# lbcb-sci/raven

Hardware: AMD Instinct MI355X
Metric: read Gbase/s through overlap+polish (higher is better)
Workload: dtype u32

## Files before the change

raven_amd/csrc/poa4.hip:

```cpp
#include <algorithm>
#include <cstddef>
#include <cstdio>
#include <cstdlib>
#include <cstring>
#include <vector>

#include "poa.h"
#include "poa2_window.h"

namespace rvn {

namespace {

struct P4 {
  static constexpr int G = 4, GS = 16, kBand = 32;
  static constexpr int kRing = 22;
  static constexpr int kRowB = 64;
  static constexpr int kMaxD = 8;
  static constexpr int kEdges = 8;
  static constexpr int kEdgesMax = 15;
  static constexpr int kU = 8;
};
constexpr u32 kNone4 = 0xFFFFu;
constexpr i32 kNegU = -0x30000000;
// ... 93 lines not shown
__host__ __device__ __forceinline__ i32 sext16(u32 x) { return static_cast<i32>(static_cast<i16>(x & 0xFFFFu)); }
__host__ __device__ __forceinline__ i32 imax(i32 a, i32 b) { return a > b ? a : b; }
__host__ __device__ __forceinline__ i32 imin(i32 a, i32 b) { return a < b ? a : b; }
template <bool HI>
__host__ __device__ __forceinline__ u32 add_half(u32 a, u32 p) {
#if defined(__HIP_DEVICE_COMPILE__)
  u32 d;
  if constexpr (HI)
    asm("v_add_u32_sdwa %0, %1, %2 dst_sel:DWORD dst_unused:UNUSED_PAD src0_sel:DWORD src1_sel:WORD_1" : "=v"(d) : "v"(a), "v"(p));
  else
    asm("v_add_u32_sdwa %0, %1, %2 dst_sel:DWORD dst_unused:UNUSED_PAD src0_sel:DWORD src1_sel:WORD_0" : "=v"(d) : "v"(a), "v"(p));
  return d;
#else
  return a + (HI ? p >> 16 : p & 0xFFFFu);
#endif
}
template <bool HI, int TAG>
__host__ __device__ __forceinline__ i32 cell_key(u32 w) {
#if defined(__HIP_DEVICE_COMPILE__)
  i32 d;
  if constexpr (HI) asm("v_mad_i32_i16 %0, %1, %2, %3 op_sel:[1,0,0,0]" : "=v"(d) : "v"(w), "s"(256), "n"(TAG));
  else asm("v_mad_i32_i16 %0, %1, %2, %3" : "=v"(d) : "v"(w), "s"(256), "n"(TAG));
  return d;
#else
  return static_cast<i32>(static_cast<i16>((HI ? w >> 16 : w) & 0xFFFFu)) * 256 + TAG;
#endif
}
__host__ __device__ __forceinline__ u32 keys_to_pair(i32 k0, i32 k1) {
#if defined(__HIP_DEVICE_COMPILE__)
  return __builtin_amdgcn_perm(static_cast<u32>(k1), static_cast<u32>(k0), 0x06050201u);
#else
  return ((static_cast<u32>(k0) >> 8) & 0xFFFFu) | ((static_cast<u32>(k1) >> 8) << 16);
#endif
}
__host__ __device__ __forceinline__ i32 imax3(i32 a, i32 b, i32 c) {
  const i32 m = a > b ? a : b;
  return m > c ? m : c;
}
template <int B>
__host__ __device__ __forceinline__ u32 put_byte(u32 acc, u32 v) {
#if defined(__HIP_DEVICE_COMPILE__)
  constexpr u32 sel = B == 0 ? 0x0C0C0C04u : (B == 1 ? 0x0C0C0400u : (B == 2 ? 0x0C040100u : 0x04020100u));
  return __builtin_amdgcn_perm(v, acc, sel);
#else
  const u32 keep = B == 0 ? 0u : (B == 1 ? 0xFFu : (B == 2 ? 0xFFFFu : 0xFFFFFFu));
  return (acc & keep) | ((v & 0xFFu) << (8 * B));
#endif
}
__host__ __device__ __forceinline__ u32 pack16(i32 lo, i32 hi) {
#if defined(__HIP_DEVICE_COMPILE__)
  return __builtin_amdgcn_perm(static_cast<u32>(hi), static_cast<u32>(lo), 0x05040100u);
#else
  return (static_cast<u32>(lo) & 0xFFFFu) | (static_cast<u32>(hi) << 16);
#endif
}
__host__ __device__ __forceinline__ u32 clamp_pair(u32 w) {
#if defined(__HIP_DEVICE_COMPILE__)
  typedef short pk16 __attribute__((ext_vector_type(2)));
  const pk16 lim = {static_cast<short>(kNegInf16), static_cast<short>(kNegInf16)};
  return __builtin_bit_cast(u32, __builtin_elementwise_max(__builtin_bit_cast(pk16, w), lim));
#else
  const i32 a = sext16(w), b = sext16(w >> 16);
  return pack16(a < kNegInf16 ? kNegInf16 : a, b < kNegInf16 ? kNegInf16 : b);
#endif
}
__host__ __device__ __forceinline__ u32 lds_ld32(const Poa4Lds& S, u32 off) {
  return *reinterpret_cast<const u32*>(reinterpret_cast<const unsigned char*>(&S) + off);
}
__host__ __device__ __forceinline__ void lds_st32(Poa4Lds& S, u32 off, u32 v) {
  *reinterpret_cast<u32*>(reinterpret_cast<unsigned char*>(&S) + off) = v;
}
__host__ __device__ __forceinline__ i32 lds_ld16(const Poa4Lds& S, u32 off) {
  return *reinterpret_cast<const i16*>(reinterpret_cast<const unsigned char*>(&S) + off);
}
__host__ __device__ __forceinline__ void lds_order() {
#if defined(__HIP_DEVICE_COMPILE__)
  __builtin_amdgcn_wave_barrier();
#else
  sv::sync();
#endif
}
#if defined(__HIP_DEVICE_COMPILE__)
#define P4_MARK(x) asm volatile("; P4MARK " x)
#define P4_ASSUME_GLOBAL(p) \
  __builtin_assume(!__builtin_amdgcn_is_shared((const void*)(p))); \
  __builtin_assume(!__builtin_amdgcn_is_private((const void*)(p)))
#define P4_ASSUME_LDS(p) __builtin_assume(__builtin_amdgcn_is_shared((const void*)(p)))
#else
#define P4_MARK(x)
#define P4_ASSUME_GLOBAL(p)
#define P4_ASSUME_LDS(p)
#endif

__host__ __device__ __forceinline__ unsigned char* opaque(unsigned char* p) {
#if defined(__HIP_DEVICE_COMPILE__)
  asm volatile("" : "+v"(p));
#endif
  return p;
}

__host__ __device__ inline u32 group_min_u(u32 v) {
#pragma unroll
  for (int off = 8; off > 0; off >>= 1) {
    const u32 o = static_cast<u32>(sv::bperm(static_cast<int>(v), sv::lane() ^ off));
    v = o < v ? o : v;
  }
  return v;
}
__host__ __device__ inline i32 group_max_i(i32 v) {
#pragma unroll
  for (int off = 8; off > 0; off >>= 1) {
    const i32 o = sv::bperm(v, sv::lane() ^ off);
    v = o > v ? o : v;
  }
  return v;
}

__host__ __device__ inline u32 poa4_nth_pred_rank(const Poa4Slot& sl, u32 v, u32 k, bool full) {
  const Poa2Slot& g = sl.g;
  const u32 c = g.in_cnt[v];
  u32 seen = 0;
  for (u32 i = 0; i < c; ++i) {
    const u32 t = g.in_tail[v * kPoaMaxIn + i];
    if (full || g.mark[t]) {
      if (seen == k) return sl.rb[t] & 0xFFFFu;
      ++seen;
    }
  }
  return 0;
}

__host__ __device__ __forceinline__ u32 mulhi_u32(u32 a, u32 b) {
#if defined(__HIP_DEVICE_COMPILE__)
  return __umulhi(a, b);
#else
  return static_cast<u32>((static_cast<unsigned long long>(a) * b) >> 32);
#endif
}
__host__ __device__ __forceinline__ u32 magic_of(u32 d) { return d <= 1 ? 0u : static_cast<u32>(0x100000000ULL / d) + 1u; }
__host__ __device__ __forceinline__ u32 div_magic(u32 n, u32 m) { return m ? mulhi_u32(n, m) : n; }

struct alignas(16) Poa4LdsDesc {
  u32 segtab[32];
  u32 seq2[60];
  u8 bytes[1024];
};

__host__ __device__ inline void poa4_guide_to_lds(Poa4LdsDesc& S, const PoaLayer* Lp, u32 len, i32 span) {
  const int lane = sv::lane();
  if (lane < 8) {
    const i32 sg = lane;
    const i32 x0 = (sg * span) / 8, x1 = ((sg + 1) * span) / 8;
    const i32 wa = sg == 0 ? 0 : static_cast<i32>(Lp->way[sg - 1]);
    const i32 wb = sg == 7 ? static_cast<i32>(len) : static_cast<i32>(Lp->way[sg]);
    S.segtab[4 * sg] = static_cast<u32>(x0);
    S.segtab[4 * sg + 1] = static_cast<u32>(wa);
    S.segtab[4 * sg + 2] = static_cast<u32>(wb - wa);
    S.segtab[4 * sg + 3] = magic_of(static_cast<u32>(x1 > x0 ? x1 - x0 : 1));
  }
}
template <class K>
__host__ __device__ __forceinline__ i32 poa4_band_start(const Poa4LdsDesc& S, i32 bpos, i32 lb, i32 span, u32 span_magic, u32 len) {
  i32 x = bpos - lb;
  x = x < 0 ? 0 : (x > span ? span : x);
  const u32 seg = div_magic(static_cast<u32>(x) * 8u, span_magic);
  const u32 sg = seg > 7u ? 7u : seg;
  const uint4 st = *reinterpret_cast<const uint4*>(&S.segtab[4 * sg]);
  const i32 dw = static_cast<i32>(st.z);
  const u32 num = static_cast<u32>(x - static_cast<i32>(st.x)) * static_cast<u32>(dw < 0 ? -dw : dw);
  const i32 qn = static_cast<i32>(div_magic(num, st.w));
  i32 b = static_cast<i32>(st.y) + (dw < 0 ? -qn : qn) - K::kBand / 2;
  const i32 bmax = static_cast<i32>(len) + 1 - K::kBand;
// ... 749 lines not shown
              g.al[static_cast<size_t>(kt[u][k]) * 4 + ac[u]] = static_cast<u16>(id);
              g.al_cnt[kt[u][k]] = static_cast<u8>(ac[u] + 1);
              if (c2 == 0) mine.x = kt[u][k];
              else if (c2 == 1) mine.x |= kt[u][k] << 16;
              else mine.y = kt[u][k];
              ++c2;
            }
          }
          if (ac[u] < 4) {
            g.al[static_cast<size_t>(an[u]) * 4 + ac[u]] = static_cast<u16>(id);
            g.al_cnt[an[u]] = static_cast<u8>(ac[u] + 1);
          }
          if (c2 == 0) mine.x = an[u];
          else if (c2 == 1) mine.x |= an[u] << 16;
          else if (c2 == 2) mine.y = an[u];
          else mine.y |= an[u] << 16;
          ++c2;
        }
        *reinterpret_cast<uint2*>(g.al + static_cast<size_t>(id) * 4) = mine;
        g.al_cnt[id] = static_cast<u8>(c2);
      }
      if (why == 0) total_new += cnt;
      tgt[u] = t;
    }
    u32 icnt[UP];
    uint4 ta[UP], tb[UP];
#pragma unroll
    for (int u = 0; u < UP; ++u) {
      const bool old = valid[u] && why == 0 && !is_new[u];
      const u32 t = old ? tgt[u] : 0u;
      icnt[u] = old ? g.in_cnt[t] : 0u;
      ta[u] = old ? *reinterpret_cast<const uint4*>(g.in_tail + static_cast<size_t>(t) * kPoaMaxIn) : uint4{0, 0, 0, 0};
      tb[u] = old ? *reinterpret_cast<const uint4*>(g.in_tail + static_cast<size_t>(t) * kPoaMaxIn + 8) : uint4{0, 0, 0, 0};
    }
#pragma unroll
    for (int u = 0; u < UP; ++u) {
      const u32 last_t = static_cast<u32>(sv::bperm(static_cast<int>(u == 0 ? prev_tgt : tgt[u > 0 ? u - 1 : 0]), gbase | (GW - 1)));
      const i32 last_w = sv::bperm(u == 0 ? prev_w : wgt[u > 0 ? u - 1 : 0], gbase | (GW - 1));
      const u32 tail = static_cast<u32>(shift1(static_cast<int>(tgt[u]), static_cast<int>(last_t)));
      const i32 tw = shift1(wgt[u], last_w);
      if (valid[u] && why == 0) {
        const u32 head = tgt[u];
        if (len >= 2) {
          if (is_new[u]) g.visits[head] = 1;
          else atomic_inc_u16(g.visits, head);
        }
        if (p[u] >= 1) {
          const i32 weight = tw + wgt[u];
          const u32 c = icnt[u];
          u32 found = 0xFFu;
#pragma unroll
          for (int i2 = 0; i2 < 16; ++i2) {
            const uint4& src4 = i2 < 8 ? ta[u] : tb[u];
            const u32 wd = (i2 & 7) < 2 ? src4.x : ((i2 & 7) < 4 ? src4.y : ((i2 & 7) < 6 ? src4.z : src4.w));
            const u32 tt = (wd >> (16 * (i2 & 1))) & 0xFFFFu;
            if (static_cast<u32>(i2) < c && tt == tail && found == 0xFFu) found = static_cast<u32>(i2);
          }
          if (found != 0xFFu) {
            atomic_add_i32(g.in_w + static_cast<size_t>(head) * kPoaMaxIn + found, weight);
          } else if (c >= static_cast<u32>(kPoaMaxIn)) {
            why = 3;
          } else {
            g.in_tail[static_cast<size_t>(head) * kPoaMaxIn + c] = static_cast<u16>(tail);
            g.in_w[static_cast<size_t>(head) * kPoaMaxIn + c] = weight;
            g.in_cnt[head] = static_cast<u8>(c + 1);
            atomic_inc_u16(g.out_cnt, tail);
          }
        }
      }
    }
    {
      const u32 wmax = static_cast<u32>(gmax(static_cast<i32>(why)));
      why = wmax;
    }
    prev_tgt = static_cast<u32>(sv::bperm(static_cast<int>(tgt[UP - 1]), gbase | (GW - 1)));
    prev_w = sv::bperm(wgt[UP - 1], gbase | (GW - 1));
  }
  t_add += sv::clock() - t0;
  t0 = sv::clock();
  const u32 n_new = total_new;
  lds_order();
  const bool doit = act && why == 0 && n_new != 0;
  if (sv::any(doit)) {
    const u32 max_old = static_cast<u32>(sv::wave_max(doit ? static_cast<int>(n_old) : 0));
    for (u32 r0 = 0; r0 < max_old; r0 += UP * GW) {
      u32 rr[UP], vv[UP];
#pragma unroll
      for (int u = 0; u < UP; ++u) {
        rr[u] = r0 + static_cast<u32>(GW) * static_cast<u32>(u) + static_cast<u32>(gl);
        vv[u] = (doit && rr[u] < n_old) ? g.order[rr[u]] : 0u;
      }
#pragma unroll
      for (int u = 0; u < UP; ++u) {
        if (doit && rr[u] < n_old) {
          u32 lo = 0, hi = n_new;
          while (lo < hi) {
            const u32 mid = (lo + hi) >> 1;
            if (nslot[mid] <= rr[u]) lo = mid + 1;
            else hi = mid;
          }
          g.order2[rr[u] + lo] = static_cast<u16>(vv[u]);
          rb16[2 * static_cast<size_t>(vv[u])] = static_cast<u16>(rr[u] + lo);
        }
      }
    }
    const u32 max_new = static_cast<u32>(sv::wave_max(doit ? static_cast<int>(n_new) : 0));
    for (u32 t = static_cast<u32>(gl); t < max_new; t += GW) {
      if (doit && t < n_new) {
        const u32 r = static_cast<u32>(nslot[t]) + t;
        g.order2[r] = static_cast<u16>(n_old + t);
        rb16[2 * static_cast<size_t>(n_old + t)] = static_cast<u16>(r);
      }
    }
    if (doit) flip = !flip;
  }
  if (act && why == 0) nn = n_old + n_new;
  sv::sync();
  t_ord += sv::clock() - t0;
  return why;
}

__host__ __device__ inline void poa4_consensus_general(Poa2Slot& g, u32 n_nodes, u32 nmax, const PoaWindow& win, int trim, Poa4Lds& S,
                                               u8* out, u32* out_len) {
  const int lane = sv::lane();
  for (u32 r = lane; r < n_nodes; r += 64) g.rank_of[g.order[r]] = static_cast<u16>(r);
  constexpr u32 kCap = sizeof(Poa4Lds) / 4;
  i32* lsc = reinterpret_cast<i32*>(&S);
  i32 maxn = -1;
  if (n_nodes > kCap) {
    if (lane == 0) maxn = poa_consensus_scores_lane0(g, n_nodes);
    maxn = sv::rfl(maxn);
  } else {
    i32 max_sc = 0;
    const u32 nn = n_nodes;
    for (u32 r0 = 0; r0 < nn; r0 += 64) {
      const u32 rows = nn - r0 < 64 ? nn - r0 : 64;
      int m_it = 0, m_c = 0, m_t01 = 0, m_t23 = 0, m_w0 = 0, m_w1 = 0, m_w2 = 0, m_w3 = 0;
      if (static_cast<u32>(lane) < rows) {
        m_it = g.order[r0 + lane];
        m_c = g.in_cnt[m_it];
        const u16* tp = g.in_tail + static_cast<size_t>(m_it) * kPoaMaxIn;
        const i32* wp = g.in_w + static_cast<size_t>(m_it) * kPoaMaxIn;
        m_t01 = static_cast<int>(static_cast<u32>(tp[0]) | (static_cast<u32>(tp[1]) << 16));
        m_t23 = static_cast<int>(static_cast<u32>(tp[2]) | (static_cast<u32>(tp[3]) << 16));
        m_w0 = wp[0];
        m_w1 = wp[1];
        m_w2 = wp[2];
        m_w3 = wp[3];
      }
      for (u32 l = 0; l < rows; ++l) {
        const int li = static_cast<int>(l);
        const u32 it = static_cast<u32>(sv::rl(m_it, li));
        const u32 c = static_cast<u32>(sv::rl(m_c, li));
        const u32 t01 = static_cast<u32>(sv::rl(m_t01, li)), t23 = static_cast<u32>(sv::rl(m_t23, li));
        const i32 w0 = sv::rl(m_w0, li), w1 = sv::rl(m_w1, li), w2 = sv::rl(m_w2, li), w3 = sv::rl(m_w3, li);
        i32 sc = -1, pd = -1, pd_sc = 0;
        for (u32 k = 0; k < c; ++k) {
          i32 wgt, t;
          if (k < 4) {
            t = static_cast<i32>(((k < 2 ? t01 : t23) >> (16 * (k & 1))) & 0xFFFFu);
            wgt = k == 0 ? w0 : (k == 1 ? w1 : (k == 2 ? w2 : w3));
          } else {
            wgt = g.in_w[static_cast<size_t>(it) * kPoaMaxIn + k];
            t = static_cast<i32>(g.in_tail[static_cast<size_t>(it) * kPoaMaxIn + k]);
          }
          const i32 st = lsc[t];
          if (sc < wgt || (sc == wgt && pd_sc <= st)) {
            sc = wgt;
            pd = t;
            pd_sc = st;
          }
        }
        if (pd != -1) sc += pd_sc;
        lds_order();
        if (lane == 0) {
          lsc[it] = sc;
          g.scores[it] = sc;
          g.preds[it] = pd;
        }
        lds_order();
        if (maxn == -1 || max_sc < sc) {
          maxn = static_cast<i32>(it);
          max_sc = sc;
        }
      }
    }
  }
  sv::sync();
  u32 cl = 0;
  i32 begin = 0, end = -1;
  if (lane == 0) poa_consensus_trace_lane0(g, n_nodes, nmax, win, trim, maxn, &cl, &begin, &end);
  cl = static_cast<u32>(sv::rfl(static_cast<int>(cl)));
  begin = sv::rfl(begin);
  end = sv::rfl(end);
  sv::sync();
  i32 n_out = end - begin + 1;
  if (n_out < 0) n_out = 0;
  if (static_cast<u32>(n_out) > win.out_cap) n_out = static_cast<i32>(win.out_cap);
  for (i32 p = lane; p < n_out; p += 64) out[p] = g.code[g.stack[cl - 1 - static_cast<u32>(begin + p)]];
// ... 358 lines not shown
    me.phase = kFailed;
    me.status = 4;
    if (lane == 0) C.st[rec] = me;
    return;
  }
  const Poa4Slot sl = poa4_carve(poa4_slot_of(A, C, wave_dp, q), A.nmax, A.lmax);
  Poa2Slot g = sl.g;
  for (u32 i = lane; i < L.len; i += 64) {
    S.bytes[i] = static_cast<u8>(poa_layer_code(A.src, L, i));
    g.pos_node[i] = static_cast<u16>(kNone4);
  }
  lds_order();
  if (lane < 60) {
    u32 x = 0;
    for (u32 c = 0; c < 16; ++c) {
      const i32 p = static_cast<i32>(static_cast<u32>(lane) * 16 + c) - 1;
      if (p >= 0 && p < static_cast<i32>(L.len)) x |= static_cast<u32>(S.bytes[p] & 3u) << (2 * c);
    }
    sl.seq2g[lane] = x;
  }
  const u32 blen = A.layers[wq.layer_first].len;
  const u32 offset = static_cast<u32>(0.01 * blen);
  const bool full = L.begin < offset && L.end > blen - offset;
  u32 r_lo = 0, r_hi = me.nn;
  if (!full) {
    lds_order();
    poa4_subgraph_marks(g, sl.rb, me.flip ? g.order2 : g.order, reinterpret_cast<u32*>(S.bytes), me.nn, L.begin, L.end, r_lo, r_hi);
  }
  const i32 lb = static_cast<i32>(L.begin), span = static_cast<i32>(L.end) - static_cast<i32>(L.begin) + 1;
  poa4_guide_to_lds(S, A.layers + wq.layer_first + liq, L.len, span);
  lds_order();
  if (lane < 32) sl.seq2g[64 + lane] = S.segtab[lane];
  u32 b_first = 0;
  if (r_hi > r_lo) {
    const u32 v0 = (me.flip ? g.order2 : g.order)[r_lo];
    b_first = static_cast<u32>(poa4_band_start<K>(S, static_cast<i32>(sl.rb[v0] >> 16), lb, span,
                                                   magic_of(static_cast<u32>(span > 0 ? span : 1)), L.len));
  }
  me.act = 1;
  me.full = full ? 1u : 0u;
  me.len = L.len;
  me.lb = L.begin;
  me.span = static_cast<u32>(span);
  me.r_lo = r_lo;
  me.n_rows = r_hi - r_lo;
  me.t_end = 0;
  me.best_rho1 = 0;
  me.b_first = b_first;
  me.dflag = 0;
  if (lane == 0) C.st[rec] = me;
  if (A.phase_cycles && lane == 0) sv::atomic_add(&A.phase_cycles[0], sv::clock() - t0);
}

constexpr int kDescPer = 4;
template <class K>
__host__ __device__ inline void poa4_phase_desc_onewave(const Poa4Args& A, const Poa4Ctx& C, Poa4LdsDesc& S, u32 rec) {
  const int lane = sv::lane();
  const u32 wave_dp = rec / P4::G;
  const int q = static_cast<int>(rec % P4::G);
  if (poa4_my_record(C, wave_dp, q) == 0xFFFFFFFFu) return;
  const Poa4Slot sl = poa4_carve(poa4_slot_of(A, C, wave_dp, q), A.nmax, A.lmax);
  const Poa2Slot& g = sl.g;
  const Poa4Win me = C.st[rec];
  if (me.phase != kRunning || !me.act) return;
  const unsigned long long t_desc0 = sv::clock();
  const u32 nn = me.nn;
  const bool full = me.full != 0;
  const u32 len = me.len, r_lo = me.r_lo, n_rows = me.n_rows, r_hi = r_lo + n_rows;
  const i32 lb = static_cast<i32>(me.lb), span = static_cast<i32>(me.span), b_first = static_cast<i32>(me.b_first);
  const u32 span_magic = magic_of(static_cast<u32>(span > 0 ? span : 1));
  const u32 dump_off = poa4_dump_byte(q);
  const u32 neg_off = poa4_neg_byte(q);
  const u32 neg2 = neg_off | (neg_off << 16);
  u32 flag = 0, marked_rows = 0;
  i32 t_end = 0;
  {
    const u32 gw = sl.seq2g[lane < 60 ? lane : 64 + (lane - 60)];
    const u32 gw2 = lane < 28 ? sl.seq2g[68 + lane] : 0u;
    if (lane < 60) S.seq2[lane] = gw;
    else S.segtab[lane - 60] = gw;
    if (lane < 28) S.segtab[4 + lane] = gw2;
  }
  lds_order();
  for (u32 v0 = 0; v0 < nn; v0 += 64 * kDescPer) {
    u32 rbv[kDescPer];
#pragma unroll
    for (int u = 0; u < kDescPer; ++u) {
      const u32 v = v0 + static_cast<u32>(u) * 64 + static_cast<u32>(lane);
      rbv[u] = v < nn ? sl.rb[v] : 0u;
    }
#pragma unroll
    for (int u = 0; u < kDescPer; ++u) {
      const u32 v = v0 + static_cast<u32>(u) * 64 + static_cast<u32>(lane);
      if (v < nn) {
        const i32 b = poa4_band_start<K>(S, static_cast<i32>(rbv[u] >> 16), lb, span, span_magic, len);
        sl.rbl[v] = (rbv[u] & 0xFFFFu) | (static_cast<u32>(b) << 16);
      }
    }
  }
  sv::sync();
  for (u32 v0 = 0; v0 < nn; v0 += 64 * kDescPer) {
    u32 vv[kDescPer], rbv[kDescPer], cc[kDescPer], code[kDescPer], outc_f[kDescPer], outc_s[kDescPer], mk[kDescPer];
    uint4 tl[kDescPer];
#pragma unroll
    for (int u = 0; u < kDescPer; ++u) {
      vv[u] = v0 + static_cast<u32>(u) * 64 + static_cast<u32>(lane);
      const u32 vq = vv[u] < nn ? vv[u] : 0u;
      rbv[u] = sl.rbl[vq];
      cc[u] = g.in_cnt[vq];
      code[u] = g.code[vq];
      outc_f[u] = g.out_cnt[vq];
      outc_s[u] = full ? 0u : g.sub_out[vq];
      mk[u] = full ? 1u : g.mark[vq];
      tl[u] = *reinterpret_cast<const uint4*>(g.in_tail + static_cast<size_t>(vq) * kPoaMaxIn);
    }
    bool ok[kDescPer], marked[kDescPer];
    u32 cmax = 0;
#pragma unroll
    for (int u = 0; u < kDescPer; ++u) {
      const u32 r = rbv[u] & 0xFFFFu;
      ok[u] = vv[u] < nn && r >= r_lo && r < r_hi;
      marked[u] = ok[u] && mk[u] != 0;
      if (!marked[u]) cc[u] = 0;
      cmax = cc[u] > cmax ? cc[u] : cmax;
    }
    cmax = static_cast<u32>(sv::wave_max(static_cast<i32>(cmax)));
    u32 trb[kDescPer][8], tmk[kDescPer][8];
#pragma unroll
    for (int k = 0; k < 8; ++k) {
      if (static_cast<u32>(k) < cmax) {
#pragma unroll
        for (int u = 0; u < kDescPer; ++u) {
          const u32 wd = k < 2 ? tl[u].x : (k < 4 ? tl[u].y : (k < 6 ? tl[u].z : tl[u].w));
          const u32 t = static_cast<u32>(k) < cc[u] ? (wd >> (16 * (k & 1))) & 0xFFFFu : 0u;
          trb[u][k] = sl.rbl[t];
          tmk[u][k] = full ? 1u : g.mark[t];
        }
      } else {
#pragma unroll
        for (int u = 0; u < kDescPer; ++u) {
          trb[u][k] = 0;
          tmk[u][k] = 0;
        }
      }
    }
#pragma unroll
    for (int u = 0; u < kDescPer; ++u) {
      const u32 v = vv[u];
      const u32 r = rbv[u] & 0xFFFFu;
      const i32 b = static_cast<i32>(rbv[u] >> 16);
      const u32 rho = r - r_lo;
      u32 ep[4] = {neg2, neg2, neg2, neg2};
      u32 np = 0, lbw = 0, lbk7 = 0;
      auto edge = [&](u32 rbt, bool inside) {
        if (!inside) return;
        const u32 lbk = r - (rbt & 0xFFFFu);
        const i32 d = b - static_cast<i32>(rbt >> 16);
        if (lbk < 1 || lbk > static_cast<u32>(K::kRing - 1) || lbk > rho || d < 0 || d > K::kMaxD) {
          flag = 7;
        } else if (np < static_cast<u32>(K::kEdges)) {
          const u32 e = poa4_ring_byte(q, ((rho - lbk) % static_cast<u32>(K::kRing)) * static_cast<u32>(kRowW4));
          const u32 idx = np >> 1;
          const u32 keep = (np & 1) ? 0x0000FFFFu : 0xFFFF0000u;
          const u32 put = (np & 1) ? e << 16 : e;
#pragma unroll
          for (u32 i = 0; i < 4; ++i) ep[i] = i == idx ? ((ep[i] & keep) | put) : ep[i];
          if (np < 6) lbw |= lbk << (5 * np);
          if (np == 7) lbk7 = lbk;
        } else if (np < static_cast<u32>(K::kEdgesMax)) {
          const u32 e = poa4_ring_byte(q, ((rho - lbk) % static_cast<u32>(K::kRing)) * static_cast<u32>(kRowW4));
          u16* const o16 = reinterpret_cast<u16*>(sl.ovf + rho);
          if (np == static_cast<u32>(K::kEdges)) {
            sl.ovf[rho] = uint4{(ep[3] >> 16) | (neg_off << 16), neg2, neg2, neg2};
            ep[3] = (ep[3] & 0xFFFFu) | (neg_off << 16);
            if (lbk7 > static_cast<u32>(K::kRing - 2)) flag = 7;
          }
          o16[np - 7] = static_cast<u16>(e);
          if (lbk > static_cast<u32>(K::kRing - 2)) flag = 7;
        }
        ++np;
      };
#pragma unroll
// ... 366 lines not shown
      }
      sv::sync();
      if (!any_layer) break;
      poa4_phase_nw<K, SC>(A, C, S.u.n, pw);
      sv::phase_fence();
    }
    poa4_phase_final(A, C, S.u.f, pw);
    sv::phase_fence();
  }
}

template <int UP, class SC>
__global__ __launch_bounds__(64) __attribute__((amdgpu_waves_per_eu(4, 4))) void poa4_persistent_kernel(const Poa4Args A, const Poa4Ctx C) {
  __shared__ Poa4LdsAll lds;
  poa4_persistent<P4, UP, SC>(A, C, lds, blockIdx.x);
}
__host__ __device__ inline bool poa4_racon_scores(const Poa4Args& A) {
  return A.m == Poa4ScoresRacon::m && A.n_ == Poa4ScoresRacon::n && A.gp == Poa4ScoresRacon::g;
}

Poa4Args args_of4(const PoaBatchDev& b, unsigned char* scratch, size_t slot_bytes) {
  Poa4Args A{};
  A.windows = b.wins;
  A.n_windows = b.n_windows;
  A.layers = b.layers;
  A.src = b.src;
  A.scratch = scratch;
  A.slot_bytes = slot_bytes;
  A.nmax = b.nmax;
  A.lmax = b.lmax;
  A.m = b.m;
  A.n_ = b.n;
  A.gp = b.g;
  A.trim = b.trim;
  A.out = b.out;
  A.out_len = b.out_len;
  A.status = b.status;
  A.phase_cycles = b.phase_cycles;
  A.sched = b.sched;
  A.next = b.next;
  A.esc = nullptr;
  A.esc_cap = 0;
  A.esc_wide = 0;
  return A;
}

}

void poa_v4_launch(Engine& e, const PoaBatchDev& b) {
  if (b.n_windows == 0) return;
  const size_t slot_bytes = poa4_slot_bytes(b.nmax, b.lmax);
  int dev = 0, cus = 256;
  RVN_HIP(hipGetDevice(&dev));
  RVN_HIP(hipDeviceGetAttribute(&cus, hipDeviceAttributeMultiprocessorCount, dev));
  u32 gw = b.n_windows > 2u * static_cast<u32>(cus) * 16u ? static_cast<u32>(P4::G) : 2u;
  if (const char* ev = knob("RVN_POA_GW")) gw = std::min<u32>(P4::G, std::max(1, std::atoi(ev)));
  const u32 n_quads = (b.n_windows + gw - 1) / gw;
  size_t free_b = 0, total_b = 0;
  RVN_HIP(hipMemGetInfo(&free_b, &total_b));
  const size_t per_wave = P4::G * (slot_bytes + sizeof(Poa4Win));
  const size_t budget = std::max(e.poa2_scratch.cap, devpool::free_largest()) + free_b / 2;
  u32 n_waves = std::min<u32>(n_quads, static_cast<u32>(cus) * 16u);
  if (static_cast<size_t>(n_waves) * per_wave + 1024 > budget) n_waves = static_cast<u32>(std::max<size_t>(1, (budget - 1024) / per_wave));
  const size_t slots = static_cast<size_t>(n_waves) * P4::G;
  unsigned char* d_scratch = e.poa2_scratch.get<unsigned char>(slots * (slot_bytes + sizeof(Poa4Win)) + 512);
  Poa4Win* d_st = reinterpret_cast<Poa4Win*>(d_scratch + slots * slot_bytes + 256);
  Poa4Args A = args_of4(b, d_scratch, slot_bytes);
  if (b.esc && poa2_slot_bytes(b.nmax, b.lmax, 64) <= P4::G * slot_bytes) {
    A.esc = b.esc;
    A.esc_cap = b.esc_cap;
    A.esc_wide = poa2_slot_bytes(b.nmax, b.lmax, 128) <= P4::G * slot_bytes ? 1u : 0u;
  }
  hipStream_t s = e.stream;
  RVN_HIP(hipMemsetAsync(b.next, 0, 4, s));
  const Poa4Ctx C{d_st, 0, b.n_windows, 0, gw};
  if (poa4_racon_scores(A)) {
    RVN_KLAUNCH_ON(kKPoaRows, s, (poa4_persistent_kernel<kUpdPer, Poa4ScoresRacon><<<n_waves, 64, 0, s>>>(A, C)));
  } else {
    RVN_KLAUNCH_ON(kKPoaRows, s, (poa4_persistent_kernel<kUpdPer, Poa4ScoresAny><<<n_waves, 64, 0, s>>>(A, C)));
  }
}

#ifdef RVN_TEST_HOOKS
namespace {
struct EmuCall4 {
  const Poa4Args* A;
  const Poa4Ctx* C;
  Poa4Lds* S;
  Poa4LdsGraph* SG;
  Poa4LdsNw* SN;
  Poa4LdsAll* SA;
  u32 wave;
  int phase;
};
void emu_entry4(void* p) {
  EmuCall4* c = static_cast<EmuCall4*>(p);
  switch (c->phase) {
    case 0: poa4_phase_init(*c->A, *c->C, c->wave); break;
    case 1: poa4_phase_graph<P4, kUpdPer>(*c->A, *c->C, *c->SG, c->wave); break;
    case 2:
      if (poa4_racon_scores(*c->A)) poa4_phase_nw<P4, Poa4ScoresRacon>(*c->A, *c->C, *c->SN, c->wave);
      else poa4_phase_nw<P4, Poa4ScoresAny>(*c->A, *c->C, *c->SN, c->wave);
      break;
    case 9:
      if (poa4_racon_scores(*c->A)) poa4_persistent<P4, kUpdPer, Poa4ScoresRacon>(*c->A, *c->C, *c->SA, c->wave);
      else poa4_persistent<P4, kUpdPer, Poa4ScoresAny>(*c->A, *c->C, *c->SA, c->wave);
      break;
    default: poa4_phase_final(*c->A, *c->C, *c->S, c->wave); break;
  }
}
}

void poa_v4_emulate(const std::vector<PoaWindow>& wins, const std::vector<PoaLayer>& lays, const PoaSrc& src, u32 max_bb,
                    u32 max_len, int m, int n, int g, int trim, u8* out, u32* out_len, u32* status, bool persistent) {
  if (wins.empty()) return;
  PoaBatchDev b{};
  b.lmax = std::min<u32>(kPoaMaxSeq, std::max<u32>(64, ((max_len + 63) / 64) * 64));
  b.nmax = std::min<u32>(8192, std::max<u32>(512, max_bb * 6));
  const size_t slot_bytes = poa4_slot_bytes(b.nmax, b.lmax);
  const u32 count = static_cast<u32>(wins.size());
  const u32 n_waves = (count + P4::G - 1) / P4::G;
  std::vector<unsigned char> scratch(slot_bytes * std::max<u32>(n_waves, 2) * P4::G + 256, 0);
  std::vector<Poa4Win> st(static_cast<size_t>(std::max<u32>(n_waves, 2)) * P4::G);
  unsigned long long phase[16] = {};
  u32 next = 0;
  b.wins = wins.data();
  b.n_windows = count;
  b.layers = lays.data();
  b.src = src;
  b.m = m;
  b.n = n;
  b.g = g;
  b.trim = trim;
  b.out = out;
  b.out_len = out_len;
  b.status = status;
  b.phase_cycles = phase;
  b.sched = nullptr;
  b.next = &next;
  const Poa4Args A = args_of4(b, scratch.data(), slot_bytes);
  const Poa4Ctx C{st.data(), 0, count, 0};
  std::vector<Poa4Lds> lds(1);
  std::vector<Poa4LdsGraph> ldsg(1);
  std::vector<Poa4LdsNw> ldsn(1);
  if (persistent) {
    std::vector<Poa4LdsAll> ldsa(1);
    const Poa4Ctx CP{st.data(), 0, count, 0};
    for (u32 pw : {1u, 0u}) {
      std::memset(static_cast<void*>(ldsa.data()), 0, sizeof(Poa4LdsAll));
      EmuCall4 call{&A, &CP, lds.data(), ldsg.data(), ldsn.data(), ldsa.data(), pw, 9};
      simt_emu::run_wave(&emu_entry4, &call);
    }
    return;
  }
  u32 max_layers = 0;
  for (const PoaWindow& w : wins) max_layers = std::max(max_layers, w.n_layers);
  auto run = [&](int ph) {
    const u32 waves = ph == 1 ? n_waves * P4::G : n_waves;
    for (u32 wv = 0; wv < waves; ++wv) {
      if (ph == 1 && (wv >= count || st[wv].phase != kRunning)) continue;
      std::memset(static_cast<void*>(lds.data()), 0, sizeof(Poa4Lds));
      std::memset(static_cast<void*>(ldsg.data()), 0, sizeof(Poa4LdsGraph));
      std::memset(static_cast<void*>(ldsn.data()), 0, sizeof(Poa4LdsNw));
      EmuCall4 call{&A, &C, lds.data(), ldsg.data(), ldsn.data(), nullptr, wv, ph};
      simt_emu::run_wave(&emu_entry4, &call);
    }
  };
  run(0);
  for (u32 round = 1; round <= max_layers; ++round) {
    run(1);
    if (round < max_layers) run(2);
  }
  run(5);
}

#endif

}
```

raven_amd/hip.py:

```python
from __future__ import annotations

import ctypes as C
import os

import numpy as np

_HERE = os.path.dirname(os.path.abspath(__file__))
LIB_PATH = os.environ.get("RVN_LIB_PATH") or os.path.join(_HERE, "lib", "libraven_hip.so")
TEST_LIB_PATH = os.path.join(os.path.dirname(LIB_PATH), "libraven_hip_test.so")

OVERLAP_DTYPE = np.dtype([
    ("lhs_id", "<u4"), ("lhs_begin", "<u4"), ("lhs_end", "<u4"),
    ("rhs_id", "<u4"), ("rhs_begin", "<u4"), ("rhs_end", "<u4"),
    ("score", "<u4"), ("strand", "<u4")])

ED_PAIR_DTYPE = np.dtype([
    ("lhs_read", "<u4"), ("lhs_begin", "<u4"), ("lhs_len", "<u4"),
    ("rhs_read", "<u4"), ("rhs_begin", "<u4"), ("rhs_len", "<u4"),
    ("strand", "<u4"), ("reserved", "<u4")])

ALIGN_PAIR_DTYPE = np.dtype([
    ("query_read", "<u4"), ("query_begin", "<u4"), ("query_len", "<u4"),
    ("target_read", "<u4"), ("target_begin", "<u4"), ("target_len", "<u4"),
    ("strand", "<u4"), ("reserved", "<u4")])
# ... 368 lines not shown
    def find_chimeric_regions(self, invalid):
        inv = np.ascontiguousarray(invalid, dtype=np.uint8)
        off = np.zeros(self.n + 1, dtype=np.uint32)
        ptr = C.c_void_p()
        _check(lib().rvn_pass1_find_chimeric_regions(self._h, _p(inv), _p(off), C.byref(ptr)))
        total = int(off[-1])
        try:
            flat = np.ctypeslib.as_array(C.cast(ptr, C.POINTER(C.c_uint32)), shape=(max(2 * total, 1),))[:2 * total].copy()
        finally:
            lib().rvn_free(ptr)
        flat = flat.reshape(-1, 2)
        return [flat[int(off[i]):int(off[i + 1])] for i in range(self.n)]

    def overlaps(self):
        L = lib()
        n = int(L.rvn_pass1_num_overlaps(self._h))
        ovl = np.zeros(n, dtype=OVERLAP_DTYPE)
        off = np.zeros(self.n + 1, dtype=np.uint32)
        _check(L.rvn_pass1_fetch_overlaps(self._h, _p(ovl), _p(off)))
        return ovl, off

    def close(self):
        if getattr(self, "_h", None):
            lib().rvn_pass1_destroy(self._h)
            self._h = None

    def __del__(self):
        try:
            self.close()
        except Exception:
            pass


def _pack_poa_windows(windows):
    codes, quals, loff, begins, ends, hasq, woff, ooff = [], [], [0], [], [], [], [0], [0]
    any_q = False
    for wdw in windows:
        layers = wdw["layers"]
        k = len(layers)
        blen = len(layers[0])
        b = wdw.get("begins") or [0] * k
        e_ = wdw.get("ends") or [max(blen - 1, 0)] * k
        q = wdw.get("quals")
        for i, lay in enumerate(layers):
            lay = np.asarray(lay, dtype=np.uint8)
            codes.append(lay)
            loff.append(loff[-1] + lay.shape[0])
            begins.append(int(b[i]))
            ends.append(int(e_[i]))
            if q is not None and q[i] is not None:
                quals.append(np.asarray(q[i], dtype=np.uint8))
                hasq.append(1)
                any_q = True
            else:
                quals.append(np.full(lay.shape[0], 33, dtype=np.uint8))
                hasq.append(0)
        woff.append(woff[-1] + k)
        ooff.append(ooff[-1] + 4 * blen + 256)
    nw = len(windows)
    return dict(codes=np.concatenate(codes) if codes else np.zeros(0, np.uint8),
                quals=np.concatenate(quals) if any_q else None, loff=np.asarray(loff, dtype=np.uint64),
                begins=np.asarray(begins, dtype=np.uint32), ends=np.asarray(ends, dtype=np.uint32),
                hasq=np.asarray(hasq, dtype=np.uint32), woff=np.asarray(woff, dtype=np.uint32), nw=nw,
                out=np.zeros(ooff[-1] + 16, dtype=np.uint8), ooff=np.asarray(ooff, dtype=np.uint64),
                out_len=np.zeros(nw, dtype=np.uint32), status=np.zeros(nw, dtype=np.uint32))


def _unpack_poa_consensus(a):
    ooff = a["ooff"]
    return [a["out"][int(ooff[i]): int(ooff[i]) + int(a["out_len"][i])].copy() for i in range(a["nw"])]


def poa_banded_emulate(windows, m=3, n=-5, g=-4, trim=True, variant=4):
    a = _pack_poa_windows(windows)
    T = test_lib()
    rc = T.rvn_poa_banded_emulate(
        _p(a["codes"]), _p(a["quals"]), _p(a["loff"]), _p(a["begins"]), _p(a["ends"]), _p(a["hasq"]), _p(a["woff"]),
        a["nw"], m, n, g, int(trim), _p(a["out"]), _p(a["ooff"]), _p(a["out_len"]), _p(a["status"]), int(variant))
    if rc != RVN_OK:
        raise (ValueError if rc == RVN_EINVAL else RavenHipError)(T.rvn_last_error().decode(errors="replace"))
    return _unpack_poa_consensus(a), a["status"]


class Engine:

    def __init__(self, k=15, w=5, bandwidth=500, chain=4, matches=100, gap=10000, device=0):
        self.k, self.w = min(max(k, 1), 31), w
        h = C.c_void_p()
        _check(lib().rvn_engine_create(C.byref(h), k, w, bandwidth, chain, matches, gap, device))
        self._h = h

    def close(self):
        if getattr(self, "_h", None):
            lib().rvn_engine_destroy(self._h)
            self._h = None

    def __del__(self):
        try:
            self.close()
        except Exception:
            pass

    def upload(self, rs) -> Reads:
        return Reads(self, rs)

    def load(self, path) -> Reads:
        h = C.c_void_p()
        st = np.zeros(8, dtype=np.uint64)
        _check(lib().rvn_reads_load(self._h, str(path).encode(), C.byref(h), _p(st)))
        n = C.c_uint32(0)
        lib().rvn_reads_info(h, C.byref(n), None, None, None, None)
        lengths = np.zeros(n.value, dtype=np.uint32)
        lib().rvn_reads_fetch(h, None, None, _p(lengths), None, None)
        rs = CodeSet(lengths)
        rs.names = [lib().rvn_reads_name(h, i).decode() for i in range(n.value)]
        r = Reads.__new__(Reads)
        r.rs, r.engine, r._h = rs, self, h
        r.load_stats = {"n_sequences": int(st[0]), "n_bases": int(st[1]), "has_quality": int(st[2] & 0xFFFFFFFF),
                        "parse_s": float(st[3:4].view(np.float64)[0]), "device_s": float(st[4:5].view(np.float64)[0]),
                        "total_s": float(st[5:6].view(np.float64)[0]), "inflate_threads": int(st[6] & 0xFFFFFFFF),
                        "members": int(st[6] >> 32), "streaming": int(st[7] & 0xFFFFFFFF), "restarted": int(st[7] >> 32)}
        return r

    def upload_codes(self, code_arrays) -> Reads:
        lens = [int(len(c)) for c in code_arrays]
        flat = np.concatenate([np.asarray(c, dtype=np.uint8) for c in code_arrays]) if lens else np.zeros(0, np.uint8)
        return Reads(self, CodeSet(lens), codes=flat)

    def polish_output_as_reads(self, lengths) -> Reads:
        h = C.c_void_p()
        _check(lib().rvn_polish_output_as_reads(self._h, C.byref(h)))
        return Reads(self, CodeSet([int(x) for x in lengths]), handle=h)

    def minimize(self, reads: Reads, first=0, last=None, minhash=False):
        last = reads.n if last is None else last
        _check(lib().rvn_engine_minimize(self._h, reads._h, first, last, int(minhash)))

    def filter(self, f):
        _check(lib().rvn_engine_filter(self._h, float(f)))

    @property
    def occurrence(self):
        return int(lib().rvn_engine_occurrence(self._h))

    def map_batch(self, reads: Reads, first=0, last=None, avoid_equal=True, avoid_symmetric=True, minhash=False,
                  want_filtered=False):
        last = reads.n if last is None else last
        n = C.c_uint64(0)
        _check(lib().rvn_engine_map_batch(self._h, reads._h, first, last, int(avoid_equal), int(avoid_symmetric),
                                          int(minhash), int(want_filtered), C.byref(n)))
        ovl = np.zeros(n.value, dtype=OVERLAP_DTYPE)
        off = np.zeros(last - first + 1, dtype=np.uint32)
        _check(lib().rvn_engine_map_fetch(self._h, _p(ovl), _p(off)))
        res = dict(overlaps=ovl, read_offsets=off)
        if want_filtered:
            tot = C.c_uint64(0)
            _check(lib().rvn_engine_map_fetch_filtered(self._h, None, None, C.byref(tot)))
            pos = np.zeros(tot.value, dtype=np.uint32)
            foff = np.zeros(last - first + 1, dtype=np.uint32)
            _check(lib().rvn_engine_map_fetch_filtered(self._h, _p(pos), _p(foff), C.byref(tot)))
            res["filtered"] = pos
            res["filtered_offsets"] = foff
        return res

    def find_overlaps_and_create_piles(self, reads: Reads, freq=0.001, kmax=32, use_minhash=False,
                                       index_batch_bases=1 << 32, flush_bases=1 << 30) -> Pass1:
# ... 743 lines not shown
```

Measured before the change: 1.411.

## Software-pipeline order merge with vectorized loads and batch band-start descriptor loads

Rewrites the topological order merge so each lane handles 16 contiguous old ranks. It loads them as two 128-bit vectors, prefetched two turns ahead, and does one binary search per chunk, then advances linearly through the inserted-slot list instead of searching once per element. The band-start descriptor pass now issues loads for four turns before computing, so more memory latency is in flight. Asm markers pin the register lifetimes. Test-only emulator hooks are added to check order consistency and report node counts. The price is higher register pressure and uncoalesced, per-lane contiguous access in the order merge.

```diff
diff --git a/raven_amd/csrc/poa4.hip b/raven_amd/csrc/poa4.hip
--- a/raven_amd/csrc/poa4.hip
+++ b/raven_amd/csrc/poa4.hip
@@ -199,12 +199,14 @@
 }
 #if defined(__HIP_DEVICE_COMPILE__)
 #define P4_MARK(x) asm volatile("; P4MARK " x)
+#define P4_MARK_USE4(x, a, b, c, d) asm volatile("; P4MARK " x : "+v"(a), "+v"(b), "+v"(c), "+v"(d))
 #define P4_ASSUME_GLOBAL(p) \
   __builtin_assume(!__builtin_amdgcn_is_shared((const void*)(p))); \
   __builtin_assume(!__builtin_amdgcn_is_private((const void*)(p)))
 #define P4_ASSUME_LDS(p) __builtin_assume(__builtin_amdgcn_is_shared((const void*)(p)))
 #else
 #define P4_MARK(x)
+#define P4_MARK_USE4(x, a, b, c, d)
 #define P4_ASSUME_GLOBAL(p)
 #define P4_ASSUME_LDS(p)
 #endif
@@ -1120,30 +1122,63 @@
   lds_order();
   const bool doit = act && why == 0 && n_new != 0;
   if (sv::any(doit)) {
+    constexpr u32 kOrdPer = 16, kOrdTurn = kOrdPer * static_cast<u32>(GW);
+    typedef u32 v4u __attribute__((ext_vector_type(4)));
     const u32 max_old = static_cast<u32>(sv::wave_max(doit ? static_cast<int>(n_old) : 0));
-    for (u32 r0 = 0; r0 < max_old; r0 += UP * GW) {
-      u32 rr[UP], vv[UP];
-#pragma unroll
-      for (int u = 0; u < UP; ++u) {
-        rr[u] = r0 + static_cast<u32>(GW) * static_cast<u32>(u) + static_cast<u32>(gl);
-        vv[u] = (doit && rr[u] < n_old) ? g.order[rr[u]] : 0u;
-      }
-#pragma unroll
-      for (int u = 0; u < UP; ++u) {
-        if (doit && rr[u] < n_old) {
-          u32 lo = 0, hi = n_new;
-          while (lo < hi) {
-            const u32 mid = (lo + hi) >> 1;
-            if (nslot[mid] <= rr[u]) lo = mid + 1;
-            else hi = mid;
+    u32 og = static_cast<u32>(gl);
+#if defined(__HIP_DEVICE_COMPILE__)
+    asm volatile("" : "+v"(og));
+#endif
+    auto ord_load = [&](u32 r0, v4u& a, v4u& b) __attribute__((always_inline)) {
+      const u32 rb0 = r0 + kOrdPer * og;
+      a = (doit && rb0 < n_old) ? *reinterpret_cast<const v4u*>(g.order + rb0) : v4u{0, 0, 0, 0};
+      b = (doit && rb0 + 8 < n_old) ? *reinterpret_cast<const v4u*>(g.order + rb0 + 8) : v4u{0, 0, 0, 0};
+    };
+    auto ord_store = [&](u32 r0, const v4u& a, const v4u& b) __attribute__((always_inline)) {
+      const u32 rb0 = r0 + kOrdPer * og;
+      if (doit && rb0 < n_old) {
+        u32 lo = 0, hi = n_new;
+        while (lo < hi) {
+          const u32 mid = (lo + hi) >> 1;
+          if (nslot[mid] <= rb0) lo = mid + 1;
+          else hi = mid;
+        }
+        u32 nxt = lo < n_new ? nslot[lo] : 0xFFFFFFFFu;
+#pragma unroll
+        for (u32 k = 0; k < kOrdPer; ++k) {
+          const u32 r = rb0 + k;
+          if (r < n_old) {
+            while (nxt <= r) {
+              ++lo;
+              nxt = lo < n_new ? nslot[lo] : 0xFFFFFFFFu;
+            }
+            const v4u& src = k < 8 ? a : b;
+            const u32 wd = (k & 7) < 2 ? src.x : ((k & 7) < 4 ? src.y : ((k & 7) < 6 ? src.z : src.w));
+            const u32 v = (wd >> (16 * (k & 1))) & 0xFFFFu;
+            g.order2[r + lo] = static_cast<u16>(v);
+            rb16[2 * static_cast<size_t>(v)] = static_cast<u16>(r + lo);
           }
-          g.order2[rr[u] + lo] = static_cast<u16>(vv[u]);
-          rb16[2 * static_cast<size_t>(vv[u])] = static_cast<u16>(rr[u] + lo);
-        }
-      }
-    }
+        }
+      }
+    };
+    v4u oa0, ob0, oa1, ob1;
+    ord_load(0, oa0, ob0);
+    ord_load(kOrdTurn, oa1, ob1);
+    u32 r0 = 0;
+    for (; r0 + 2 * kOrdTurn < max_old; r0 += kOrdTurn) {
+      v4u oa2, ob2;
+      ord_load(r0 + 2 * kOrdTurn, oa2, ob2);
+      ord_store(r0, oa0, ob0);
+      oa0 = oa1;
+      ob0 = ob1;
+      oa1 = oa2;
+      ob1 = ob2;
+    }
+    P4_MARK_USE4("ord_store_begin", oa0, ob0, oa1, ob1);
+    ord_store(r0, oa0, ob0);
+    ord_store(r0 + kOrdTurn, oa1, ob1);
     const u32 max_new = static_cast<u32>(sv::wave_max(doit ? static_cast<int>(n_new) : 0));
-    for (u32 t = static_cast<u32>(gl); t < max_new; t += GW) {
+    for (u32 t = og; t < max_new; t += GW) {
       if (doit && t < n_new) {
         const u32 r = static_cast<u32>(nslot[t]) + t;
         g.order2[r] = static_cast<u16>(n_old + t);
@@ -1153,6 +1188,7 @@
     if (doit) flip = !flip;
   }
   if (act && why == 0) nn = n_old + n_new;
+  P4_MARK("ord_store_end");
   sv::sync();
   t_ord += sv::clock() - t0;
   return why;
@@ -1677,22 +1713,32 @@
     if (lane < 28) S.segtab[4 + lane] = gw2;
   }
   lds_order();
-  for (u32 v0 = 0; v0 < nn; v0 += 64 * kDescPer) {
-    u32 rbv[kDescPer];
-#pragma unroll
-    for (int u = 0; u < kDescPer; ++u) {
-      const u32 v = v0 + static_cast<u32>(u) * 64 + static_cast<u32>(lane);
-      rbv[u] = v < nn ? sl.rb[v] : 0u;
-    }
-#pragma unroll
-    for (int u = 0; u < kDescPer; ++u) {
-      const u32 v = v0 + static_cast<u32>(u) * 64 + static_cast<u32>(lane);
-      if (v < nn) {
-        const i32 b = poa4_band_start<K>(S, static_cast<i32>(rbv[u] >> 16), lb, span, span_magic, len);
-        sl.rbl[v] = (rbv[u] & 0xFFFFu) | (static_cast<u32>(b) << 16);
-      }
-    }
-  }
+  static_assert(kDescPer == 4, "the turn marker takes the turn's four words");
+  constexpr int kDesc1Turns = 4;
+  P4_MARK("desc1_begin");
+  for (u32 c0 = 0; c0 < nn; c0 += 64 * kDescPer * kDesc1Turns) {
+    u32 rbv[kDesc1Turns][kDescPer];
+#pragma unroll
+    for (int t = 0; t < kDesc1Turns; ++t) {
+#pragma unroll
+      for (int u = 0; u < kDescPer; ++u) {
+        const u32 v = c0 + static_cast<u32>(t * kDescPer + u) * 64 + static_cast<u32>(lane);
+        rbv[t][u] = sl.rb[v < nn ? v : nn - 1];
+      }
+    }
+#pragma unroll
+    for (int t = 0; t < kDesc1Turns; ++t) {
+      if (c0 + static_cast<u32>(t * kDescPer) * 64 >= nn) break;
+      P4_MARK_USE4("desc1_turn", rbv[t][0], rbv[t][1], rbv[t][2], rbv[t][3]);
+#pragma unroll
+      for (int u = 0; u < kDescPer; ++u) {
+        const u32 v = c0 + static_cast<u32>(t * kDescPer + u) * 64 + static_cast<u32>(lane);
+        const i32 b = poa4_band_start<K>(S, static_cast<i32>(rbv[t][u] >> 16), lb, span, span_magic, len);
+        sl.rbl[v < nn ? v : nn - 1] = (rbv[t][u] & 0xFFFFu) | (static_cast<u32>(b) << 16);
+      }
+    }
+  }
+  P4_MARK("desc1_end");
   sv::sync();
   for (u32 v0 = 0; v0 < nn; v0 += 64 * kDescPer) {
     u32 vv[kDescPer], rbv[kDescPer], cc[kDescPer], code[kDescPer], outc_f[kDescPer], outc_s[kDescPer], mk[kDescPer];
@@ -2225,6 +2271,13 @@
 }
 
 #ifdef RVN_TEST_HOOKS
+}
+constexpr unsigned kEmuReportWindows = 64;
+extern "C" {
+uint32_t rvn_test_poa_emulate_max_nodes[kEmuReportWindows] = {};
+uint64_t rvn_test_poa_emulate_order_violations = 0;
+}
+namespace rvn {
 namespace {
 struct EmuCall4 {
   const Poa4Args* A;
@@ -2236,6 +2289,22 @@
   u32 wave;
   int phase;
 };
+void emu_check_orders(const Poa4Args& A, const Poa4Ctx& C, const std::vector<Poa4Win>& st, u32 count) {
+  for (u32 wv = 0; wv < count; ++wv) {
+    const Poa4Win& w = st[wv];
+    if (w.phase != kRunning && w.phase != kLayersDone) continue;
+    unsigned char* slot = poa4_slot_of(A, C, wv / P4::G, static_cast<int>(wv % P4::G));
+    const Poa2Slot g = poa4_graph(slot, A.nmax, A.lmax, w.flip != 0);
+    const u32* rb = poa4_carve(slot, A.nmax, A.lmax).rb;
+    if (wv < kEmuReportWindows) rvn_test_poa_emulate_max_nodes[wv] = std::max(rvn_test_poa_emulate_max_nodes[wv], w.nn);
+    for (u32 v = 0; v < w.nn; ++v) {
+      const u32 r = rb[v] & 0xFFFFu;
+      if (r >= w.nn || g.order[r] != v) ++rvn_test_poa_emulate_order_violations;
+      for (u32 k = 0; k < g.in_cnt[v]; ++k)
+        if ((rb[g.in_tail[static_cast<size_t>(v) * kPoaMaxIn + k]] & 0xFFFFu) >= r) ++rvn_test_poa_emulate_order_violations;
+    }
+  }
+}
 void emu_entry4(void* p) {
   EmuCall4* c = static_cast<EmuCall4*>(p);
   switch (c->phase) {
@@ -2286,6 +2355,8 @@
   std::vector<Poa4Lds> lds(1);
   std::vector<Poa4LdsGraph> ldsg(1);
   std::vector<Poa4LdsNw> ldsn(1);
+  std::memset(rvn_test_poa_emulate_max_nodes, 0, sizeof(rvn_test_poa_emulate_max_nodes));
+  rvn_test_poa_emulate_order_violations = 0;
   if (persistent) {
     std::vector<Poa4LdsAll> ldsa(1);
     const Poa4Ctx CP{st.data(), 0, count, 0};
@@ -2312,6 +2383,7 @@
   run(0);
   for (u32 round = 1; round <= max_layers; ++round) {
     run(1);
+    emu_check_orders(A, C, st, count);
     if (round < max_layers) run(2);
   }
   run(5);
diff --git a/raven_amd/hip.py b/raven_amd/hip.py
--- a/raven_amd/hip.py
+++ b/raven_amd/hip.py
@@ -474,6 +474,12 @@
     return _unpack_poa_consensus(a), a["status"]
 
 
+def poa_emulate_graph_report():
+    T = test_lib()
+    nodes = np.array((C.c_uint32 * 64).in_dll(T, "rvn_test_poa_emulate_max_nodes"), dtype=np.uint32)
+    return nodes, int(C.c_uint64.in_dll(T, "rvn_test_poa_emulate_order_violations").value)
+
+
 class Engine:
 
     def __init__(self, k=15, w=5, bandwidth=500, chain=4, matches=100, gap=10000, device=0):
```

New measurement: 1.433, median of 6. +1.6%, better.
